# muelea/tuch

Hardware: AMD Instinct MI355X
Metric: SMPLify-DC fit iters/sec at batch 64 (higher is better)
Workload: dtype f32; 1 GPU; configs[1] extended to the full stage-2 step: batch=64/GPU SMPL forward + contact_fitting_loss (L_P/L_C push/pull, winding inside test, segment filter, r2r) + backward + Adam, V=6890 F=13776, float32; bodies_per_gpu=64, global_batch=64, launch=hipGraph replay of the whole step

## Files before the change

tuch_amd/csrc/ray_winding.hip:

```cpp
#include "common.h"
#include "model.h"
#include "workspace.h"
#include "tree_device.h"
#include <stdlib.h>

#pragma clang fp contract(off)

namespace {

constexpr float kPi = 3.14159265358979323846f;
constexpr int kBlock = 256;
constexpr int kRayQueries = 64;
constexpr float kShearX = 0.3217f, kShearY = 0.4331f;
constexpr float kFanX = 0.8191f, kFanY = 0.3467f, kFanZ = 0.4571f;
constexpr int kSlabs = 9;
constexpr int kSlabStride = 10;
constexpr int kNearSlabs = 13;

struct RayElem { float x, y, z, sign; };

__device__ __forceinline__ float shear_x(float x, float z) { return __builtin_fmaf(-kShearX, z, x); }
__device__ __forceinline__ float shear_y(float y, float z) { return __builtin_fmaf(-kShearY, z, y); }

__global__ __launch_bounds__(kBlock) void ray_stream_kernel(
// ... 1 lines not shown
    int V, int L, int Lpad, RayElem* __restrict__ out, uint4* __restrict__ zeroed, size_t zeroed_n)
{
    const int b = blockIdx.y;
    const int p = blockIdx.x * kBlock + threadIdx.x;
    for (size_t g = ((size_t)b * gridDim.x + blockIdx.x) * kBlock + threadIdx.x; g < zeroed_n;
         g += (size_t)gridDim.x * gridDim.y * kBlock)
        zeroed[g] = make_uint4(0u, 0u, 0u, 0u);
    if (p >= Lpad) return;
    RayElem e = {0.f, 0.f, 0.f, 0.f};
    if (p < L) {
        const float* c = verts + ((size_t)b * V + vidx[p]) * 3;
        e.x = shear_x(c[0], c[2]); e.y = shear_y(c[1], c[2]); e.z = c[2]; e.sign = sign[p];
    }
    out[(size_t)b * Lpad + p] = e;
}

__device__ __forceinline__ void slab_project(float x, float y, float z, float (&p)[kSlabs])
{
    p[0] = x; p[1] = y; p[2] = z;
    p[3] = x + y; p[4] = x - y; p[5] = x + z; p[6] = x - z; p[7] = y + z; p[8] = y - z;
}

template <int kCtrl>
__device__ __forceinline__ float dpp_move(float x)
{
    return __int_as_float(__builtin_amdgcn_update_dpp(0, __float_as_int(x), kCtrl, 0xF, 0xF, true));
}
__device__ __forceinline__ float row_min(float v)
{
    v = fminf(v, dpp_move<0xB1>(v));
    v = fminf(v, dpp_move<0x4E>(v));
    v = fminf(v, dpp_move<0x141>(v));
    v = fminf(v, dpp_move<0x140>(v));
    return v;
}

__device__ __forceinline__ uint32_t half_below(float x)
{
    const _Float16 h = (_Float16)x;
    uint32_t u = __builtin_bit_cast(uint16_t, h);
    if ((float)h > x) u = (u & 0x8000u) ? u + 1 : (u == 0 ? 0x8001u : u - 1);
    return u;
}
__device__ __forceinline__ uint32_t half_above(float x)
{
    const _Float16 h = (_Float16)x;
    uint32_t u = __builtin_bit_cast(uint16_t, h);
    if ((float)h < x) u = (u & 0x8000u) ? (u == 0x8000u ? 0x0001u : u - 1) : u + 1;
    return u;
}
__device__ __host__ __forceinline__ size_t near_records_at(int B, int L) { return (size_t)B * kNearSlabs * L; }
__device__ __host__ __forceinline__ size_t near_centres_at(int B, int L) { return near_records_at(B, L) + (size_t)B * L * 8; }

template <bool kPose>
__global__ __launch_bounds__(kBoundsBlock) void ray_leaf_bounds_kernel(
    const RayElem* __restrict__ stream, int T, const TreeNode* __restrict__ nodes, int N,
    const int32_t* __restrict__ height_off, const int32_t* __restrict__ height_nodes, float* __restrict__ bounds,
    const float* __restrict__ verts, const int32_t* __restrict__ vidx, const float* __restrict__ sign, int V, int Lexact,
    RayElem* __restrict__ stream_out, uint4* __restrict__ zeroed, size_t zeroed_n)
{
    const int b = blockIdx.y;
    const RayElem* st = stream + (size_t)b * T;
    const int group = threadIdx.x >> 4, sub = threadIdx.x & 15;
    const int i = height_off[0] + blockIdx.x * (kBoundsBlock / 16) + group;
    const bool real = i < height_off[1];
    const int node = height_nodes[real ? i : height_off[0]];
    const int off = nodes[node].ex_off, len = real ? nodes[node].ex_len : 0;
    if (kPose) {
        for (size_t g = ((size_t)b * gridDim.x + blockIdx.x) * kBoundsBlock + threadIdx.x; g < zeroed_n;
             g += (size_t)gridDim.x * gridDim.y * kBoundsBlock)
            zeroed[g] = make_uint4(0u, 0u, 0u, 0u);
        if (blockIdx.x == 0)
            for (int p = Lexact + (int)threadIdx.x; p < T; p += kBoundsBlock) stream_out[(size_t)b * T + p] = RayElem{0.f, 0.f, 0.f, 0.f};
    }
    float lo[kSlabs], nhi[kSlabs];
#pragma unroll
    for (int k = 0; k < kSlabs; ++k) { lo[k] = 3.0e38f; nhi[k] = 3.0e38f; }
    for (int p = sub; p < len; p += 16) {
        RayElem e;
        if (kPose) {
            const float* c = verts + ((size_t)b * V + vidx[off + p]) * 3;
            e.x = shear_x(c[0], c[2]); e.y = shear_y(c[1], c[2]); e.z = c[2]; e.sign = sign[off + p];
            stream_out[(size_t)b * T + off + p] = e;
        } else {
            e = st[off + p];
        }
        float pr[kSlabs];
        slab_project(e.x, e.y, e.z, pr);
#pragma unroll
        for (int k = 0; k < kSlabs; ++k) { lo[k] = fminf(lo[k], pr[k]); nhi[k] = fminf(nhi[k], -pr[k]); }
    }
#pragma unroll
    for (int k = 0; k < kSlabs; ++k) { lo[k] = row_min(lo[k]); nhi[k] = row_min(nhi[k]); }
    if (real && sub == 0) {
        const int L = height_off[1] - height_off[0], leaf = i - height_off[0];
        float lo_p[kSlabs], hi_p[kSlabs];
#pragma unroll
        for (int k = 0; k < kSlabs; ++k) {
            const float hi = -nhi[k];
            const float pad = 4e-7f * fmaxf(fabsf(lo[k]), fabsf(hi)) + 1e-9f;
            lo_p[k] = lo[k] - pad;
            hi_p[k] = hi + pad;
        }
        float c[3];
        if (kPose) {
            const float* c0 = verts + ((size_t)b * V + vidx[0]) * 3;
            c[0] = shear_x(c0[0], c0[2]); c[1] = shear_y(c0[1], c0[2]); c[2] = c0[2];
        } else {
            const RayElem e0 = st[0];
            c[0] = e0.x; c[1] = e0.y; c[2] = e0.z;
        }
        float pc[kSlabs];
        slab_project(c[0], c[1], c[2], pc);
        uint32_t lo_h[kSlabs], hi_h[kSlabs];
#pragma unroll
        for (int k = 0; k < kSlabs; ++k) {
            const float pad = 4e-6f * (fabsf(lo_p[k]) + fabsf(hi_p[k]) + fabsf(pc[k])) + 1e-7f;
            lo_h[k] = half_below(lo_p[k] - pc[k] - pad);
            hi_h[k] = half_above(hi_p[k] - pc[k] + pad);
        }
        uint4* r = reinterpret_cast<uint4*>(bounds + near_records_at(gridDim.y, L)) + ((size_t)b * L + leaf) * 2;
        r[0] = make_uint4(lo_h[0] | lo_h[1] << 16, lo_h[3] | lo_h[4] << 16, lo_h[6] | lo_h[8] << 16, hi_h[0] | hi_h[1] << 16);
        r[1] = make_uint4(hi_h[2] | hi_h[3] << 16, hi_h[4] | hi_h[5] << 16, hi_h[7] | (uint32_t)leaf << 16, (uint32_t)node);
        if (leaf == 0) *reinterpret_cast<float4*>(bounds + near_centres_at(gridDim.y, L) + (size_t)b * 4) = make_float4(c[0], c[1], c[2], 0.f);
    }
}

struct P3 { float x, y, z; };

__device__ __forceinline__ float edge_fn(const P3& p, const P3& q) { return p.x * q.y - p.y * q.x; }

__device__ __forceinline__ bool left_of(float e, const P3& p, const P3& q)
{
    return e > 0.0f || (e == 0.0f && (p.x < q.x || (p.x == q.x && p.y < q.y)));
}

__device__ __forceinline__ int crossing(const P3& a, const P3& b, const P3& c, float ea, float eb, float ec)
{
    const bool la = left_of(ea, b, c), lb = left_of(eb, c, a), lc = left_of(ec, a, b);
    const bool pos = la && lb && lc, neg = !la && !lb && !lc;
    if (!(pos || neg)) return 0;
    const float numz = ea * a.z + eb * b.z + ec * c.z;
    if (pos) return numz > 0.0f ? 1 : 0;
    return numz < 0.0f ? -1 : 0;
}

__device__ __forceinline__ int crossing_mostly_generic(const P3& a, const P3& b, const P3& c, float ea, float eb, float ec)
{
    const float numz = ea * a.z + eb * b.z + ec * c.z;
    const float mn = __builtin_fminf(__builtin_fminf(ea, eb), ec), mx = __builtin_fmaxf(__builtin_fmaxf(ea, eb), ec);
    int n = (int)(__builtin_fminf(mn, numz) > 0.0f) - (int)(__builtin_fmaxf(mx, numz) < 0.0f);
    const bool tie = (mn * mx == 0.0f) & (numz != 0.0f);
    if (__builtin_amdgcn_ballot_w64(tie)) {
        if (tie) n = crossing(a, b, c, ea, eb, ec);
    }
    return n;
}

template <bool kSkipIncident>
__device__ __forceinline__ int crossing_with_ties(const P3 a, const P3 b, const P3 c, float ea, float eb, float ec)
{
    if (kSkipIncident) {
        const bool za = (a.x == 0.0f) & (a.y == 0.0f) & (a.z == 0.0f);
        const bool zb = (b.x == 0.0f) & (b.y == 0.0f) & (b.z == 0.0f);
        const bool zc = (c.x == 0.0f) & (c.y == 0.0f) & (c.z == 0.0f);
        if (za | zb | zc) return 0;
    }
    return crossing(a, b, c, ea, eb, ec);
}

constexpr uint32_t kSegBias = 0x80808080u;
struct S3 { v2f xy; float z; };
__device__ __forceinline__ float edge_fn(const S3& p, const S3& q)
{
    v2f r;
    asm("v_pk_mul_f32 %0, %1, %2 op_sel:[0,1] op_sel_hi:[1,0]" : "=v"(r) : "v"(p.xy), "v"(q.xy));
    float d;
    asm("v_sub_f32 %0, %1, %2" : "=v"(d) : "v"(r.x), "v"(r.y));
    return d;
}
__device__ __forceinline__ P3 p3(const S3& a) { return P3{a.xy.x, a.xy.y, a.z}; }

template <int A, bool kSkipIncident, bool kSeg>
__device__ __forceinline__ void ray_step(const RayElem el, S3 (&s)[3], float (&e)[3], v2f qxy, float qz, int& count,
                                         int qmask, uint32_t& pa, uint32_t& pb)
{
    constexpr int Bq = (A + 1) % 3, Cq = (A + 2) % 3;
    s[A].xy = (v2f){el.x, el.y} - qxy;
    s[A].z = el.z - qz;
    e[Bq] = edge_fn(s[Cq], s[A]);
    e[Cq] = edge_fn(s[A], s[Bq]);
    const int word = __float_as_int(el.sign);
    if ((word & 0xffffff) != 0) {
        const float numz = __builtin_fmaf(e[A], s[A].z, __builtin_fmaf(e[Cq], s[Cq].z, e[Bq] * s[Bq].z));
        const float mn = __builtin_fminf(__builtin_fminf(e[0], e[1]), e[2]);
        const float mx = __builtin_fmaxf(__builtin_fmaxf(e[0], e[1]), e[2]);
        int c = (int)(__builtin_fminf(mn, numz) > 0.0f) - (int)(__builtin_fmaxf(mx, numz) < 0.0f);
        const bool edge_zero = mn * mx == 0.0f;
        if (__builtin_amdgcn_ballot_w64(edge_zero)) {
            const bool tie = edge_zero & (numz != 0.0f);
            if (__builtin_amdgcn_ballot_w64(tie)) {
                if (tie) c = crossing_with_ties<kSkipIncident>(p3(s[Bq]), p3(s[Cq]), p3(s[A]), e[Bq], e[Cq], e[A]);
            }
        }
        asm("v_mad_i32_i24 %0, %1, %2, %0" : "+v"(count) : "v"(c), "s"(word));
        if (kSeg && ((uint32_t)word >> 24) != 0) {
            const uint32_t t = ((uint32_t)word >> 24) & (uint32_t)qmask;
            if (__builtin_amdgcn_ballot_w64((t != 0) & (c != 0))) {
                uint32_t cs;
                asm("v_mul_i32_i24 %0, %1, %2" : "=v"(cs) : "v"(c), "s"(word));
                pa += cs * (((t & 15u) * 0x00204081u) & 0x01010101u);
                pb += cs * ((((t >> 4) & 15u) * 0x00204081u) & 0x01010101u);
            }
        }
    }
}

template <bool kSkipIncident, bool kSeg>
__device__ __forceinline__ void ray_run(const RayElem* __restrict__ st, int off, int len,
                                        S3 (&s)[3], float (&e)[3], v2f qxy, float qz, int& count,
                                        int qmask, uint32_t& pa, uint32_t& pb)
{
    const RayElem* p = st + off;
    RayElem n0 = p[0], n1 = p[1], n2 = p[2];
    for (int left = len; left > 0; left -= 3, p += 3) {
        asm("" : "+s"(left));
        const RayElem e0 = n0, e1 = n1, e2 = n2;
        n0 = p[3]; n1 = p[4]; n2 = p[5];
        ray_step<0, kSkipIncident, kSeg>(e0, s, e, qxy, qz, count, qmask, pa, pb);
        ray_step<1, kSkipIncident, kSeg>(e1, s, e, qxy, qz, count, qmask, pa, pb);
        ray_step<2, kSkipIncident, kSeg>(e2, s, e, qxy, qz, count, qmask, pa, pb);
    }
}

constexpr int kFallbackChunks = 8;

__device__ __forceinline__ float wave_min(float v) { return wave_min_uniform(v); }
__device__ __forceinline__ float wave_max(float v) { return wave_max_uniform(v); }


__device__ __forceinline__ float lo_minus(uint32_t s, float q)
{
    float d;
    asm("v_fma_mix_f32 %0, %1, 1.0, -%2 op_sel_hi:[1,0,0]" : "=v"(d) : "v"(s), "v"(q));
    return d;
}
__device__ __forceinline__ float hi_minus(uint32_t s, float q)
{
    float d;
    asm("v_fma_mix_f32 %0, %1, 1.0, -%2 op_sel:[1,0,0] op_sel_hi:[1,0,0]" : "=v"(d) : "v"(s), "v"(q));
    return d;
}
__device__ __forceinline__ float minus_lo(float q, uint32_t s)
{
    float d;
    asm("v_fma_mix_f32 %0, -%1, 1.0, %2 op_sel_hi:[1,0,0]" : "=v"(d) : "v"(s), "v"(q));
    return d;
}
__device__ __forceinline__ float minus_hi(float q, uint32_t s)
{
    float d;
    asm("v_fma_mix_f32 %0, -%1, 1.0, %2 op_sel:[1,0,0] op_sel_hi:[1,0,0]" : "=v"(d) : "v"(s), "v"(q));
    return d;
}
__device__ __forceinline__ float max3(float a, float b, float c)
{
    float d;
    asm("v_max3_f32 %0, %1, %2, %3" : "=v"(d) : "v"(a), "v"(b), "v"(c));
    return d;
}

template <bool kVerts, int kWaves>
__global__ __launch_bounds__(64 * kWaves) void ray_near_kernel(
    const float* __restrict__ pts, const TreeNode* __restrict__ nodes, const float* __restrict__ bounds, int N,
    int num_leaves, const int32_t* __restrict__ qperm,
    const int32_t* __restrict__ counts, int Q, int qblocks, RayEntry* __restrict__ lists, int32_t* __restrict__ list_len,
    int32_t* __restrict__ leaf_cnt,
    unsigned long long* __restrict__ stats)
{
    __builtin_amdgcn_s_setprio(3);
    const int qb = blockIdx.x, b = blockIdx.y, lane = threadIdx.x & 63;
    const int wave = kWaves > 1 ? __builtin_amdgcn_readfirstlane(threadIdx.x >> 6) : 0;
    __shared__ uint4 queue[64 * kWaves][2];
    __shared__ float range[16];
// ... 237 lines not shown
    const bool overflow = total_pairs > cap || total_tiles > max_tiles;
    if (lane == 0 && blockIdx.y == 0) body[b] = RayBody{overflow ? fallback_tiles : total_tiles, overflow ? 1 : 0};
    if (overflow) return;
    {
        int off = sp - npairs, tile = st - ntile;
        for (int l = l0; l < l1; ++l) {
            const int c = cnt[l];
            off_s[l] = off;
            tile_s[l] = tile;
            off += c;
            tile += (c + 63) >> 6;
        }
        int ent = sq - nent;
        for (int q = q0; q < q1; ++q) { blk[q] = ent; ent += len[q]; }
        if (lane == 0) blk[qblocks] = total;
    }
    __syncthreads();
    for (int l = (int)blockIdx.y + (int)gridDim.y * lane; l < num_leaves; l += (int)gridDim.y * 64) {
        const TreeNode nd = nodes[leaf_nodes[l]];
        const int ex_off = nd.ex_off, ex_len = nd.ex_len;
        const int c = cnt[l], off = off_s[l];
        RayTile* out = tiles + (size_t)b * max_tiles + tile_s[l];
        for (int k = 0; k < c; k += 64) *out++ = RayTile{ex_off, ex_len, off + k, min(64, c - k)};
    }
    int32_t* fill = leaf_fill + (size_t)b * num_leaves;
    int32_t* out = pairs + (size_t)b * cap;
    for (int base = (int)blockIdx.y * 64; base < total; base += (int)gridDim.y * 64) {
        const int g = base + lane;
        RayEntry e = RayEntry{0, 0, 0u, 0u};
        int dst = 0, qb = 0;
        if (g < total) {
            int lo = 0, hi = qblocks;
            while (hi - lo > 1) {
                const int mid = (lo + hi) >> 1;
                if (blk[mid] <= g) lo = mid; else hi = mid;
            }
            qb = lo;
            e = lists[((size_t)b * qblocks + qb) * list_stride + (g - blk[qb])];
            dst = off_s[e.leaf] + atomicAdd(&fill[e.leaf], __builtin_popcount(e.mask_lo) + __builtin_popcount(e.mask_hi));
        }
        const int m = min(64, total - base);
        for (int k = 0; k < m; ++k) {
            const uint32_t lo = __builtin_amdgcn_readlane(e.mask_lo, k), hi = __builtin_amdgcn_readlane(e.mask_hi, k);
            const int d = __builtin_amdgcn_readlane(dst, k), q = __builtin_amdgcn_readlane(qb, k);
            const unsigned long long mask = ((unsigned long long)hi << 32) | lo;
            if ((mask >> lane) & 1ull)
                out[d + __builtin_popcountll(mask & ((1ull << lane) - 1ull))] = q * kRayQueries + lane;
        }
    }
}

template <bool kVerts, bool kCount, bool kSeg>
__global__ __launch_bounds__(64) void ray_leaf_kernel(
    const float* __restrict__ pts, const RayElem* __restrict__ stream, const RayTile* __restrict__ tiles,
    const RayBody* __restrict__ body, const int32_t* __restrict__ pairs, const RayEntry* __restrict__ lists,
    const int32_t* __restrict__ list_len, const TreeNode* __restrict__ nodes, int num_leaves,
    const int32_t* __restrict__ qperm, const int32_t* __restrict__ counts, int Q, int T, int qblocks, int num_bodies,
    int cap, int max_tiles, int32_t* __restrict__ count, unsigned long long* __restrict__ stats,
    const int32_t* __restrict__ vmask, int32_t* __restrict__ seg_count)
{
    const int lane = threadIdx.x;
    struct Work { int b, off, len, slot, qmask; bool active; float qx, qy, qz; };
    int b_cur = blockIdx.x, base = 0, g = blockIdx.y;
    auto fetch = [&]() {
        Work w;
        w.b = -1; w.off = w.len = w.slot = 0; w.qmask = 0; w.active = false; w.qx = w.qy = w.qz = 0.0f;
        while (b_cur < num_bodies) {
            const int b = b_cur;
            const int nt = __builtin_amdgcn_readfirstlane(body[b].tiles);
            if (g >= base + nt) { base += nt; b_cur += gridDim.x; continue; }
            const int t = g - base;
            g += gridDim.y;
            const float* pb = pts + (size_t)b * Q * 3;
            w.b = b;
            int i0;
            if (!__builtin_amdgcn_readfirstlane(body[b].overflow)) {
                const RayTile tile = tiles[(size_t)b * max_tiles + t];
                const int n = __builtin_amdgcn_readfirstlane(tile.n), first = __builtin_amdgcn_readfirstlane(tile.first);
                w.active = lane < n;
                w.slot = pairs[(size_t)b * cap + first + (w.active ? lane : 0)];
                i0 = kVerts ? qperm[w.slot] : w.slot;
                w.off = __builtin_amdgcn_readfirstlane(tile.ex_off);
                w.len = __builtin_amdgcn_readfirstlane(tile.ex_len);
            } else {
                const int nq = kVerts ? Q : (counts ? counts[b] : Q);
                w.slot = (t / kFallbackChunks) * kRayQueries + lane;
                w.active = w.slot < nq;
                i0 = kVerts ? qperm[w.slot] : min(w.slot, nq - 1);
                w.off = t;
                w.len = -1;
            }
            w.qz = pb[3 * i0 + 2];
            w.qx = shear_x(pb[3 * i0], w.qz);
            w.qy = shear_y(pb[3 * i0 + 1], w.qz);
            if (kSeg) w.qmask = vmask[w.slot];
            break;
        }
        return w;
    };
    int walked = 0;
    Work next = fetch();
    while (next.b >= 0) {
        const Work w = next;
        next = fetch();
        S3 s[3];
        float e[3];
#pragma unroll
        for (int k = 0; k < 3; ++k) { s[k].xy = (v2f){0.0f, 0.0f}; s[k].z = 0.0f; e[k] = 0.0f; }
        const v2f qxy = {w.qx, w.qy};
        int crossings = 0;
        uint32_t pa = kSegBias, pb = kSegBias;
        const RayElem* st = stream + (size_t)w.b * T;
        if (w.len >= 0) {
            ray_run<kVerts, kSeg>(st, w.off, w.len, s, e, qxy, w.qz, crossings, w.qmask, pa, pb);
            if (kCount) walked += w.len;
        } else {
            const int qb = w.off / kFallbackChunks, c = w.off % kFallbackChunks;
            const int cnt = __builtin_amdgcn_readfirstlane(list_len[(size_t)w.b * qblocks + qb]);
            const RayEntry* list = lists + ((size_t)w.b * qblocks + qb) * num_leaves;
            for (int j = c; j < cnt; j += kFallbackChunks) {
                const TreeNode nd = nodes[__builtin_amdgcn_readfirstlane(list[j].node)];
                ray_run<kVerts, kSeg>(st, nd.ex_off, nd.ex_len, s, e, qxy, w.qz, crossings, w.qmask, pa, pb);
                if (kCount) walked += nd.ex_len;
            }
        }
        if (w.active && crossings != 0) atomicAdd(&count[((size_t)w.b * qblocks) * kRayQueries + w.slot], crossings);
        if (kSeg && w.active && (pa != kSegBias || pb != kSegBias)) {
            int32_t* sc = seg_count + 2 * (((size_t)w.b * qblocks) * kRayQueries + w.slot);
            if (pa != kSegBias) atomicAdd(sc, (int32_t)(pa - kSegBias));
            if (pb != kSegBias) atomicAdd(sc + 1, (int32_t)(pb - kSegBias));
        }
    }
    if (kCount && lane == 0) atomicAdd(stats, (unsigned long long)walked);
}

__device__ __forceinline__ float fast_atan2(float y, float x)
{
    const float ax = __builtin_fabsf(x), ay = __builtin_fabsf(y);
    const float mx = __builtin_fmaxf(__builtin_fmaxf(ax, ay), 1e-37f);
    const float t = __builtin_fminf(ax, ay) / mx;
    const float s = t * t;
    float p = 0.0024567253421992064f;
    p = p * s + -0.014401361346244812f;
    p = p * s + 0.03978123143315315f;
    p = p * s + -0.07234857976436615f;
    p = p * s + 0.10498946160078049f;
    p = p * s + -0.14161229133605957f;
    p = p * s + 0.19985906779766083f;
    p = p * s + -0.33332598209381104f;
    p = p * s + 0.9999998807907104f;
    float v = p * t;
    v = ay > ax ? 1.57079632679489661923f - v : v;
    v = x < 0.0f ? kPi - v : v;
    return __builtin_copysignf(v, y);
}

__device__ __forceinline__ float half_solid_angle(const P3& a, const P3& b, const P3& c)
{
    const float na = __builtin_sqrtf(a.x * a.x + a.y * a.y + a.z * a.z);
    const float nb = __builtin_sqrtf(b.x * b.x + b.y * b.y + b.z * b.z);
    const float nc = __builtin_sqrtf(c.x * c.x + c.y * c.y + c.z * c.z);
    const float cx = b.y * c.z - b.z * c.y, cy = b.z * c.x - b.x * c.z, cz = b.x * c.y - b.y * c.x;
    const float num = a.x * cx + a.y * cy + a.z * cz;
    const float dab = a.x * b.x + a.y * b.y + a.z * b.z;
    const float dbc = b.x * c.x + b.y * c.y + b.z * c.z;
    const float dac = a.x * c.x + a.y * c.y + a.z * c.z;
    const float den = na * nb * nc + dab * nc + dac * nb + dbc * na;
    return fast_atan2(num, den);
}

__device__ __forceinline__ void cone_term(const P3& us, const P3& sb, const P3& sc, const P3& u, const P3& pb, const P3& pc,
                                          int& crossings, float& half)
{
    const float ea = edge_fn(sb, sc), eb = edge_fn(sc, us), ec = edge_fn(us, sb);
    const float d = ea * us.z + eb * sb.z + ec * sc.z;
    const bool la = left_of(ea, sb, sc), lb = left_of(eb, sc, us), lc = left_of(ec, us, sb);
    const bool front = d >= 0.0f;
    crossings = (la & lb & lc) ? (int)front : ((!la & !lb & !lc) ? -(int)!front : 0);
    const float nu = __builtin_sqrtf(u.x * u.x + u.y * u.y + u.z * u.z);
    const float nb = __builtin_sqrtf(pb.x * pb.x + pb.y * pb.y + pb.z * pb.z);
    const float nc = __builtin_sqrtf(pc.x * pc.x + pc.y * pc.y + pc.z * pc.z);
    const float cx = pb.y * pc.z - pb.z * pc.y, cy = pb.z * pc.x - pb.x * pc.z, cz = pb.x * pc.y - pb.y * pc.x;
    const float num = __builtin_fabsf(u.x * cx + u.y * cy + u.z * cz);
// ... 319 lines not shown
        h += h1;
        c += c1;
    };
    const int e0 = active ? link_off[qq] : 0, e1 = active ? link_off[qq + 1] : 0;
    constexpr int kLongLinks = 16;
    if (e1 - e0 <= kLongLinks) {
        for (int e = e0; e < e1; e += 2) {
            int id[4];
            float pp[4][3];
#pragma unroll
            for (int u = 0; u < 4; ++u) id[u] = link[2 * min(e + (u >> 1), e1 - 1) + (u & 1)];
#pragma unroll
            for (int u = 0; u < 4; ++u) {
                const float* p = id[u] < V ? vb + 3 * (size_t)id[u] : cb + 3 * (size_t)(id[u] - V);
                pp[u][0] = p[0]; pp[u][1] = p[1]; pp[u][2] = p[2];
            }
#pragma unroll
            for (int h = 0; h < 2; ++h)
                if (e + h < e1) cone(pp[2 * h], pp[2 * h + 1], vx, vy, vz, qx, qy, half_sum, n);
        }
    }
    unsigned long long todo = __builtin_amdgcn_ballot_w64(e1 - e0 > kLongLinks);
    const int lane = threadIdx.x & 63;
    while (todo) {
        const int src = __builtin_ctzll(todo);
        todo &= todo - 1;
        const int le0 = __builtin_amdgcn_readlane(e0, src), le1 = __builtin_amdgcn_readlane(e1, src);
        const float lvx = __shfl(vx, src), lvy = __shfl(vy, src), lvz = __shfl(vz, src);
        const float lqx = __shfl(qx, src), lqy = __shfl(qy, src);
        float h = 0.0f;
        int cr = 0;
        for (int e = le0 + lane; e < le1; e += 64) {
            const int i0 = link[2 * e], i1 = link[2 * e + 1];
            const float* p0 = i0 < V ? vb + 3 * (size_t)i0 : cb + 3 * (size_t)(i0 - V);
            const float* p1 = i1 < V ? vb + 3 * (size_t)i1 : cb + 3 * (size_t)(i1 - V);
            const float a0[3] = {p0[0], p0[1], p0[2]}, a1[3] = {p1[0], p1[1], p1[2]};
            cone(a0, a1, lvx, lvy, lvz, lqx, lqy, h, cr);
        }
#pragma unroll
        for (int m = 32; m >= 1; m >>= 1) { h += __shfl_xor(h, m); cr += __shfl_xor(cr, m); }
        if (lane == src) { half_sum += h; n += cr; }
    }
    if (!active) return;
    const float w = (float)n - half_sum * (0.5f / kPi);
    const size_t o = (size_t)b * Qs_total + qq;
    if (seg_w) seg_w[o] = w;
    if (seg_ext) seg_ext[o] = w <= thresh;
    if (exterior && !(w <= thresh)) exterior[(size_t)b * V + v] = 1;
}

inline size_t align256(size_t x) { return (x + 255) & ~(size_t)255; }

struct RayLayout {
    size_t stream, bounds, lists, list_len, zeroed, zeroed_bytes, leaf_cnt, leaf_fill, count, leaf_off, tiles, body, pairs,
        stats, total;
    int T, qblocks, cap, max_tiles, workers, columns;
    size_t seg_count;
};

constexpr int kSegFusedMaxQ = 4096;
constexpr int kSegFusedMaxCaps = 8;

template <int kWaves>
__device__ __forceinline__ void seg_fused_caps(const float* __restrict__ vb, const int32_t* __restrict__ cap_off,
                                               const int32_t* __restrict__ cap_vidx, int c_lo, int c_hi, float* s_caps)
{
    const int lane = threadIdx.x & 63, wave = threadIdx.x >> 6;
    for (int c = c_lo + wave; c < c_hi; c += kWaves) {
        float sx = 0.f, sy = 0.f, sz = 0.f;
        const int beg = cap_off[c], end = cap_off[c + 1];
        for (int k = beg + lane; k < end; k += 64) {
            const float* p = vb + 3 * cap_vidx[k];
            sx += p[0]; sy += p[1]; sz += p[2];
        }
#pragma unroll
        for (int o = 32; o > 0; o >>= 1) { sx += __shfl_down(sx, o, 64); sy += __shfl_down(sy, o, 64); sz += __shfl_down(sz, o, 64); }
        if (lane == 0) {
            const float inv = 1.0f / (float)(end - beg);
            s_caps[3 * (c - c_lo)] = sx * inv; s_caps[3 * (c - c_lo) + 1] = sy * inv; s_caps[3 * (c - c_lo) + 2] = sz * inv;
        }
    }
}

constexpr int kSegOneBlock = 512, kSegOneWaves = kSegOneBlock / 64, kSegOneChunk = 256, kSegOneZ = 8;
constexpr int kSegOneOwn = kSegFusedMaxQ / kSegOneZ;
#ifdef TUCH_SEG_CLOCKS
__device__ unsigned long long g_seg_clocks[8192][8];
#define SEG_CLOCK(i) do { if (threadIdx.x == 0) { const int blk = (blockIdx.z * gridDim.y + blockIdx.y) * gridDim.x + blockIdx.x; if (blk < 8192) g_seg_clocks[blk][i] = __builtin_amdgcn_s_memrealtime(); } } while (0)
extern "C" int tuch_debug_seg_clocks(unsigned long long* out)
{
    return hipMemcpyFromSymbol(out, HIP_SYMBOL(g_seg_clocks), sizeof(unsigned long long) * 8192 * 8) == hipSuccess ? TUCH_OK : TUCH_ERR_HIP;
}
#else
#define SEG_CLOCK(i) do { } while (0)
#endif

__global__ __launch_bounds__(kSegOneBlock) void segment_one_kernel(
    const float* __restrict__ verts, const uint8_t* __restrict__ body_flags, uint8_t* __restrict__ exterior,
    const int32_t* __restrict__ seg_q_off, const int32_t* __restrict__ seg_q_vidx,
    const int32_t* __restrict__ cap_range, const int32_t* __restrict__ cap_off, const int32_t* __restrict__ cap_vidx,
    const int32_t* __restrict__ ent_off, const int32_t* __restrict__ ent,
    const int32_t* __restrict__ link_off, const int32_t* __restrict__ link, const int32_t* __restrict__ leaf_counts,
    const int32_t* __restrict__ vpos, int slots, int V, float thresh)
{
    __shared__ int32_t s_list[kSegFusedMaxQ];
    __shared__ int32_t s_cnt[kSegOneOwn];
    __shared__ float s_half[kSegOneOwn];
// ... 190 lines not shown
}

int tuch_ray_segment_flags_one(const tuch_contact_model* m, const float* verts, const uint8_t* body_flags,
                               const int32_t* leaf_counts, int B, float thresh, uint8_t* exterior, hipStream_t s)
{
    hipLaunchKernelGGL(segment_one_kernel, dim3(m->num_segments, B, kSegOneZ), dim3(kSegOneBlock), 0, s, verts, body_flags, exterior,
                       (const int32_t*)m->seg_q_off, (const int32_t*)m->seg_q_vidx, (const int32_t*)m->seg_cap_range,
                       (const int32_t*)m->cap_off, (const int32_t*)m->cap_vidx, (const int32_t*)m->seg_cap_off,
                       (const int32_t*)m->seg_cap_ent, (const int32_t*)m->seg_link_off, (const int32_t*)m->seg_link, leaf_counts,
                       (const int32_t*)m->seg_vpos, 2 * m->tree_qblocks * kRayQueries, m->V, thresh);
    return tuch_check_launch("tuch_ray_segment_flags_one");
}

bool tuch_ray_available(const tuch_contact_model* m)
{
    if (!m || m->tree_nodes <= 0 || !m->ring_off || m->tree_exact_len <= 0) return false;
    if (m->tree_leaves > 65535) return false;
    return m->opt.winding_ray != 0;
}

static int ray_pair_cap(const tuch_contact_model* m) { return m->opt.ray_pair_cap < 1 ? 1 : m->opt.ray_pair_cap; }

static RayLayout full_layout(const tuch_contact_model* m, int B, int Q, bool verts)
{
    RayLayout l;
    l.qblocks = verts ? 2 * m->tree_qblocks : ceil_div(Q, kRayQueries);
    l.T = ceil_div(m->tree_exact_len, 3) * 3 + 6;
    const int L = m->tree_leaves;
    const long cap = (long)ray_pair_cap(m) * Q;
    l.cap = (int)(cap < 0x3fffffffL ? cap : 0x3fffffffL);
    l.max_tiles = l.cap / 64 + L;
    if (l.max_tiles < l.qblocks * kFallbackChunks) l.max_tiles = l.qblocks * kFallbackChunks;
    l.columns = B < 8 ? B : 8;
    const int waves = m->opt.ray_waves > 0 ? m->opt.ray_waves : 32768;
    l.workers = waves / l.columns > 0 ? waves / l.columns : 1;
    size_t o = 0;
    l.stream = tuch_ws_take(o, (size_t)B * l.T * sizeof(RayElem));
    l.bounds = tuch_ws_take(o, (size_t)B * m->tree_nodes * 2 * kSlabStride * sizeof(float));
    l.lists = tuch_ws_take(o, (size_t)B * l.qblocks * L * sizeof(RayEntry));
    l.list_len = tuch_ws_take(o, (size_t)B * l.qblocks * sizeof(int32_t));
    l.zeroed = o;
    l.leaf_cnt = tuch_ws_take(o, (size_t)B * L * sizeof(int32_t), false);
    l.leaf_fill = tuch_ws_take(o, (size_t)B * L * sizeof(int32_t), false);
    l.count = tuch_ws_take(o, (size_t)B * l.qblocks * kRayQueries * sizeof(int32_t), false);
    l.seg_count = o;
    if (verts && m->seg_elem_mask) o += align256(2 * (size_t)B * l.qblocks * kRayQueries * sizeof(int32_t));
    l.zeroed_bytes = o - l.zeroed;
    (void)tuch_ws_take(o, 0);
    l.leaf_off = tuch_ws_take(o, (size_t)B * L * sizeof(int32_t));
    l.tiles = tuch_ws_take(o, (size_t)B * l.max_tiles * sizeof(RayTile));
    l.body = tuch_ws_take(o, (size_t)B * sizeof(RayBody));
    l.pairs = tuch_ws_take(o, (size_t)B * l.cap * sizeof(int32_t));
    l.stats = tuch_ws_take(o, 256);
    l.total = o;
    return l;
}

void tuch_ray_layout_touch(const tuch_contact_model* m, int B, int Q)
{
    (void)full_layout(m, B, Q > 0 ? Q : m->V, Q <= 0);
}

size_t tuch_ray_workspace_bytes(const tuch_contact_model* m, int B, int Q)
{
    if (!m || m->tree_nodes <= 0 || B <= 0) return 0;
    const size_t a = full_layout(m, B, m->V, true).total;
    const size_t b = Q > 0 ? full_layout(m, B, Q, false).total : 0;
    return a > b ? a : b;
}

static void launch_ray_boxes(const tuch_contact_model* m, const RayLayout& l, const float* verts, int B, char* ws, hipStream_t s,
                             bool one_launch)
{
    RayElem* st = (RayElem*)(ws + l.stream);
    float* bounds = (float*)(ws + l.bounds);
    if (one_launch && m->tree_leaf_runs_tile) {
        hipLaunchKernelGGL(ray_leaf_bounds_kernel<true>, dim3(ceil_div(m->tree_leaves, kBoundsBlock / 16), B), dim3(kBoundsBlock), 0,
                           s, (const RayElem*)st, l.T, (const TreeNode*)m->tree_node, m->tree_nodes,
                           (const int32_t*)m->tree_height_off, (const int32_t*)m->tree_height_nodes, bounds, verts,
                           (const int32_t*)m->tree_vidx, (const float*)m->tree_sign_word, m->V, m->tree_exact_len, st,
                           (uint4*)(ws + l.zeroed), l.zeroed_bytes / sizeof(uint4));
        return;
    }
    hipLaunchKernelGGL(ray_stream_kernel, dim3(ceil_div(l.T, kBlock), B), dim3(kBlock), 0, s, verts,
                       (const int32_t*)m->tree_vidx, (const float*)m->tree_sign_word, m->V, m->tree_exact_len, l.T, st,
                       (uint4*)(ws + l.zeroed), l.zeroed_bytes / sizeof(uint4));
    hipLaunchKernelGGL(ray_leaf_bounds_kernel<false>, dim3(ceil_div(m->tree_leaves, kBoundsBlock / 16), B), dim3(kBoundsBlock), 0, s,
                       (const RayElem*)st, l.T, (const TreeNode*)m->tree_node, m->tree_nodes,
                       (const int32_t*)m->tree_height_off, (const int32_t*)m->tree_height_nodes, bounds,
                       (const float*)nullptr, (const int32_t*)nullptr, (const float*)nullptr, 0, 0, (RayElem*)nullptr,
                       (uint4*)nullptr, (size_t)0);
}

template <bool kVerts>
static int launch_ray_counts(const tuch_contact_model* m, const RayLayout& l, const float* verts, const float* queries,
                             const int32_t* counts, int B, int Q, char* ws, hipStream_t s, unsigned long long* stats)
{
    launch_ray_boxes(m, l, verts, B, ws, s, kVerts);
    const int L = m->tree_leaves;
    const TreeNode* nodes = (const TreeNode*)m->tree_node;
    const int32_t* leaf_nodes = (const int32_t*)m->tree_height_nodes;
    const int32_t* qperm = kVerts ? (const int32_t*)m->tree_qperm : nullptr;
    RayEntry* lists = (RayEntry*)(ws + l.lists);
    int32_t* list_len = (int32_t*)(ws + l.list_len);
    int32_t* leaf_cnt = (int32_t*)(ws + l.leaf_cnt);
    int32_t* leaf_off = (int32_t*)(ws + l.leaf_off);
    RayTile* tiles = (RayTile*)(ws + l.tiles);
    RayBody* body = (RayBody*)(ws + l.body);
    int32_t* pairs = (int32_t*)(ws + l.pairs);
    if ((long)l.qblocks * B <= 2048)
        hipLaunchKernelGGL((ray_near_kernel<kVerts, 4>), dim3(l.qblocks, B), dim3(256), 0, s, queries, nodes,
                           (const float*)(ws + l.bounds), m->tree_nodes, L, qperm, counts, Q, l.qblocks, lists, list_len,
                           leaf_cnt, stats);
    else
        hipLaunchKernelGGL((ray_near_kernel<kVerts, 1>), dim3(l.qblocks, B), dim3(64), 0, s, queries, nodes,
                           (const float*)(ws + l.bounds), m->tree_nodes, L, qperm, counts, Q, l.qblocks, lists, list_len,
                           leaf_cnt, stats);
    const size_t tf_lds = (2 * (size_t)L + l.qblocks + 1) * sizeof(int32_t);
    if (l.qblocks <= kFillMaxBlocks && tf_lds <= 48u * 1024)
        hipLaunchKernelGGL(ray_tiles_fill_kernel, dim3(B, std::min(256, std::max(kFillSplit, 2048 / B))), dim3(kTilesFillBlock), tf_lds, s, (const int32_t*)leaf_cnt,
                           nodes, leaf_nodes, L, l.cap, l.max_tiles, l.qblocks * kFallbackChunks, tiles, body,
                           (const RayEntry*)lists, (const int32_t*)list_len, l.qblocks, (int32_t*)(ws + l.leaf_fill), pairs, L);
    else {
    hipLaunchKernelGGL(ray_tiles_kernel, dim3(B), dim3(kTilesBlock), 0, s, (const int32_t*)leaf_cnt, nodes, leaf_nodes, L, l.cap,
                       l.max_tiles, l.qblocks * kFallbackChunks, leaf_off, tiles, body);
    hipLaunchKernelGGL(ray_fill_kernel, dim3(l.qblocks, B), dim3(64), 0, s, (const RayEntry*)lists, (const int32_t*)list_len,
                       (const RayBody*)body, (const int32_t*)leaf_off, L, l.qblocks, l.cap, (int32_t*)(ws + l.leaf_fill), pairs);
    }
    const dim3 grid(l.columns, l.workers);
    const bool seg = kVerts && m->seg_elem_mask;
    const int32_t* vmask = (const int32_t*)m->seg_vmask;
    int32_t* seg_count = (int32_t*)(ws + l.seg_count);
#define TUCH_LAUNCH_RAY_LEAF(COUNT, SEG)                                                                                      \
    hipLaunchKernelGGL((ray_leaf_kernel<kVerts, COUNT, SEG>), grid, dim3(64), 0, s, queries, (const RayElem*)(ws + l.stream),  \
                       (const RayTile*)tiles, (const RayBody*)body, (const int32_t*)pairs, (const RayEntry*)lists,            \
                       (const int32_t*)list_len, nodes, L, qperm, counts, Q, l.T, l.qblocks, B, l.cap, l.max_tiles,           \
                       (int32_t*)(ws + l.count), stats, vmask, seg_count)
    if (stats) {
        if (seg) TUCH_LAUNCH_RAY_LEAF(true, kVerts); else TUCH_LAUNCH_RAY_LEAF(true, false);
    } else {
        if (seg) TUCH_LAUNCH_RAY_LEAF(false, kVerts); else TUCH_LAUNCH_RAY_LEAF(false, false);
    }
#undef TUCH_LAUNCH_RAY_LEAF
    return TUCH_OK;
}

int tuch_ray_exterior_verts(const tuch_contact_model* m, const float* verts, int B, float thresh, uint8_t* exterior,
                            float* w, void* workspace, hipStream_t s, unsigned long long* stats_host, uint8_t* exterior_copy)
{
    const RayLayout l = full_layout(m, B, m->V, true);
    char* ws = (char*)workspace;
    unsigned long long* stats = stats_host ? (unsigned long long*)(ws + l.stats) : nullptr;
    if (stats && hipMemsetAsync(stats, 0, 4 * sizeof(unsigned long long), s) != hipSuccess) return TUCH_ERR_HIP;
    const int rc = launch_ray_counts<true>(m, l, verts, verts, nullptr, B, m->V, ws, s, stats);
    if (rc != TUCH_OK) return rc;
    if (w || exterior)
        hipLaunchKernelGGL(ray_finalize_verts_kernel, dim3(ceil_div(m->V, kBlock), B), dim3(kBlock), 0, s, verts,
                           (const int32_t*)(ws + l.count), (const int32_t*)m->tree_qperm, (const int32_t*)m->ring_off,
                           (const int32_t*)m->ring_vidx, m->V, l.qblocks * kRayQueries, thresh, w, exterior, exterior_copy);
    if (stats_host) {
        RayBody bodies[8];
        const int nb = B < 8 ? B : 8;
        if (hipMemcpyAsync(stats_host, stats, 3 * sizeof(unsigned long long), hipMemcpyDeviceToHost, s) != hipSuccess ||
            hipMemcpyAsync(bodies, ws + l.body, nb * sizeof(RayBody), hipMemcpyDeviceToHost, s) != hipSuccess ||
            hipStreamSynchronize(s) != hipSuccess)
            return TUCH_ERR_HIP;
        unsigned long long tiles = 0;
        for (int b = 0; b < nb; ++b) tiles += bodies[b].tiles;
        stats_host[3] = tiles * B / nb;
    }
    return tuch_check_launch("tuch_ray_exterior_verts");
}

const int32_t* tuch_ray_segment_counts(const tuch_contact_model* m, int B, const void* workspace)
{
    if (!m->seg_elem_mask) return nullptr;
    return (const int32_t*)((const char*)workspace + full_layout(m, B, m->V, true).seg_count);
}

int tuch_ray_exterior_points(const tuch_contact_model* m, const float* verts, const float* points, const int32_t* counts,
                             int B, int Q, float thresh, uint8_t* exterior, float* w, void* workspace, hipStream_t s)
{
    const RayLayout l = full_layout(m, B, Q, false);
    char* ws = (char*)workspace;
    const int rc = launch_ray_counts<false>(m, l, verts, points, counts, B, Q, ws, s, nullptr);
    if (rc != TUCH_OK) return rc;
    hipLaunchKernelGGL(ray_finalize_points_kernel, dim3(ceil_div(Q, kBlock), B), dim3(kBlock), 0, s,
                       (const int32_t*)(ws + l.count), counts, Q, l.qblocks * kRayQueries, thresh, w, exterior);
// ... 41 lines not shown
```

Before: 152,800 body-fit iterations/s.

## Filter ray-winding triangles by 2D boxes and queue survivors for exact tests

```diff
diff --git a/tuch_amd/csrc/ray_winding.hip b/tuch_amd/csrc/ray_winding.hip
--- a/tuch_amd/csrc/ray_winding.hip
+++ b/tuch_amd/csrc/ray_winding.hip
@@ -77,12 +77,30 @@
 __device__ __host__ __forceinline__ size_t near_records_at(int B, int L) { return (size_t)B * kNearSlabs * L; }
 __device__ __host__ __forceinline__ size_t near_centres_at(int B, int L) { return near_records_at(B, L) + (size_t)B * L * 8; }
 
+constexpr float kBoxRange = 16.0f;
+constexpr float kBoxPad = 0x1p-13f;
+constexpr float kBoxSliver = 0x1p-14f;
+__device__ __forceinline__ float4 ray_elem_box(const RayElem& p0, const RayElem& p1, const RayElem& p2)
+{
+    const float inf = __builtin_inff();
+    if ((__float_as_int(p2.sign) & 0xffffff) == 0) return make_float4(inf, -inf, inf, -inf);
+    const float x0 = fminf(fminf(p0.x, p1.x), p2.x), x1 = fmaxf(fmaxf(p0.x, p1.x), p2.x);
+    const float y0 = fminf(fminf(p0.y, p1.y), p2.y), y1 = fmaxf(fmaxf(p0.y, p1.y), p2.y);
+    const float ax = p1.x - p0.x, ay = p1.y - p0.y, bx = p2.x - p0.x, by = p2.y - p0.y;
+    const float area2 = fabsf(ax * by - ay * bx);
+    const float edge = fmaxf(fmaxf(x1 - x0, y1 - y0), 0.0f);
+    const bool in_range = fmaxf(fmaxf(fabsf(x0), fabsf(x1)), fmaxf(fabsf(y0), fabsf(y1))) <= kBoxRange;
+    const bool solid = area2 > kBoxSliver * 1.4142137f * edge;
+    if (!in_range || !solid) return make_float4(-inf, inf, -inf, inf);
+    return make_float4(x0 - kBoxPad, x1 + kBoxPad, y0 - kBoxPad, y1 + kBoxPad);
+}
+
 template <bool kPose>
 __global__ __launch_bounds__(kBoundsBlock) void ray_leaf_bounds_kernel(
     const RayElem* __restrict__ stream, int T, const TreeNode* __restrict__ nodes, int N,
     const int32_t* __restrict__ height_off, const int32_t* __restrict__ height_nodes, float* __restrict__ bounds,
     const float* __restrict__ verts, const int32_t* __restrict__ vidx, const float* __restrict__ sign, int V, int Lexact,
-    RayElem* __restrict__ stream_out, uint4* __restrict__ zeroed, size_t zeroed_n)
+    RayElem* __restrict__ stream_out, uint4* __restrict__ zeroed, size_t zeroed_n, float4* __restrict__ boxes)
 {
     const int b = blockIdx.y;
     const RayElem* st = stream + (size_t)b * T;
@@ -98,18 +116,26 @@
         if (blockIdx.x == 0)
             for (int p = Lexact + (int)threadIdx.x; p < T; p += kBoundsBlock) stream_out[(size_t)b * T + p] = RayElem{0.f, 0.f, 0.f, 0.f};
     }
+    if (blockIdx.x == 0)
+        for (int p = Lexact + (int)threadIdx.x; p < T; p += kBoundsBlock)
+            boxes[(size_t)b * T + p] = make_float4(__builtin_inff(), -__builtin_inff(), __builtin_inff(), -__builtin_inff());
+    auto posed = [&](int p) {
+        RayElem e;
+        if (kPose) {
+            const float* c = verts + ((size_t)b * V + vidx[p]) * 3;
+            e.x = shear_x(c[0], c[2]); e.y = shear_y(c[1], c[2]); e.z = c[2]; e.sign = sign[p];
+        } else {
+            e = st[p];
+        }
+        return e;
+    };
     float lo[kSlabs], nhi[kSlabs];
 #pragma unroll
     for (int k = 0; k < kSlabs; ++k) { lo[k] = 3.0e38f; nhi[k] = 3.0e38f; }
     for (int p = sub; p < len; p += 16) {
-        RayElem e;
-        if (kPose) {
-            const float* c = verts + ((size_t)b * V + vidx[off + p]) * 3;
-            e.x = shear_x(c[0], c[2]); e.y = shear_y(c[1], c[2]); e.z = c[2]; e.sign = sign[off + p];
-            stream_out[(size_t)b * T + off + p] = e;
-        } else {
-            e = st[off + p];
-        }
+        const RayElem e = posed(off + p);
+        if (kPose) stream_out[(size_t)b * T + off + p] = e;
+        boxes[(size_t)b * T + off + p] = ray_elem_box(posed(off + max(p - 2, 0)), posed(off + max(p - 1, 0)), e);
         float pr[kSlabs];
         slab_project(e.x, e.y, e.z, pr);
 #pragma unroll
@@ -194,7 +220,6 @@
     return crossing(a, b, c, ea, eb, ec);
 }
 
-constexpr uint32_t kSegBias = 0x80808080u;
 struct S3 { v2f xy; float z; };
 __device__ __forceinline__ float edge_fn(const S3& p, const S3& q)
 {
@@ -206,55 +231,157 @@
 }
 __device__ __forceinline__ P3 p3(const S3& a) { return P3{a.xy.x, a.xy.y, a.z}; }
 
-template <int A, bool kSkipIncident, bool kSeg>
-__device__ __forceinline__ void ray_step(const RayElem el, S3 (&s)[3], float (&e)[3], v2f qxy, float qz, int& count,
-                                         int qmask, uint32_t& pa, uint32_t& pb)
-{
-    constexpr int Bq = (A + 1) % 3, Cq = (A + 2) % 3;
-    s[A].xy = (v2f){el.x, el.y} - qxy;
-    s[A].z = el.z - qz;
-    e[Bq] = edge_fn(s[Cq], s[A]);
-    e[Cq] = edge_fn(s[A], s[Bq]);
-    const int word = __float_as_int(el.sign);
-    if ((word & 0xffffff) != 0) {
-        const float numz = __builtin_fmaf(e[A], s[A].z, __builtin_fmaf(e[Cq], s[Cq].z, e[Bq] * s[Bq].z));
-        const float mn = __builtin_fminf(__builtin_fminf(e[0], e[1]), e[2]);
-        const float mx = __builtin_fmaxf(__builtin_fmaxf(e[0], e[1]), e[2]);
-        int c = (int)(__builtin_fminf(mn, numz) > 0.0f) - (int)(__builtin_fmaxf(mx, numz) < 0.0f);
-        const bool edge_zero = mn * mx == 0.0f;
-        if (__builtin_amdgcn_ballot_w64(edge_zero)) {
-            const bool tie = edge_zero & (numz != 0.0f);
-            if (__builtin_amdgcn_ballot_w64(tie)) {
-                if (tie) c = crossing_with_ties<kSkipIncident>(p3(s[Bq]), p3(s[Cq]), p3(s[A]), e[Bq], e[Cq], e[A]);
-            }
-        }
-        asm("v_mad_i32_i24 %0, %1, %2, %0" : "+v"(count) : "v"(c), "s"(word));
-        if (kSeg && ((uint32_t)word >> 24) != 0) {
-            const uint32_t t = ((uint32_t)word >> 24) & (uint32_t)qmask;
-            if (__builtin_amdgcn_ballot_w64((t != 0) & (c != 0))) {
-                uint32_t cs;
-                asm("v_mul_i32_i24 %0, %1, %2" : "=v"(cs) : "v"(c), "s"(word));
-                pa += cs * (((t & 15u) * 0x00204081u) & 0x01010101u);
-                pb += cs * ((((t >> 4) & 15u) * 0x00204081u) & 0x01010101u);
-            }
-        }
-    }
-}
+constexpr int kRingSize = 128;
+struct RayQueue {
+    uint32_t ring[kRingSize];
+    int32_t cross[kRayQueries];
+    uint32_t seg[2][kRayQueries];
+    float4 box[64];
+    RayElem elem[64];
+};
+constexpr int kBoxChunk = 60;
+struct RayLane { float fx, fy, qx, qy, qz; int qmask; bool active; };
 
 template <bool kSkipIncident, bool kSeg>
-__device__ __forceinline__ void ray_run(const RayElem* __restrict__ st, int off, int len,
-                                        S3 (&s)[3], float (&e)[3], v2f qxy, float qz, int& count,
-                                        int qmask, uint32_t& pa, uint32_t& pb)
-{
-    const RayElem* p = st + off;
-    RayElem n0 = p[0], n1 = p[1], n2 = p[2];
-    for (int left = len; left > 0; left -= 3, p += 3) {
-        asm("" : "+s"(left));
-        const RayElem e0 = n0, e1 = n1, e2 = n2;
-        n0 = p[3]; n1 = p[4]; n2 = p[5];
-        ray_step<0, kSkipIncident, kSeg>(e0, s, e, qxy, qz, count, qmask, pa, pb);
-        ray_step<1, kSkipIncident, kSeg>(e1, s, e, qxy, qz, count, qmask, pa, pb);
-        ray_step<2, kSkipIncident, kSeg>(e2, s, e, qxy, qz, count, qmask, pa, pb);
+__device__ __forceinline__ void ray_exact(RayQueue& q, uint32_t& head, int n, const RayLane& me, int lane)
+{
+    __syncthreads();
+    const bool valid = lane < n;
+    const uint32_t ent = q.ring[(head + (uint32_t)lane) & (kRingSize - 1)];
+    head += (uint32_t)n;
+    const int r = (int)(ent & 63u);
+    const uint32_t k = min(ent >> 6, (uint32_t)(kBoxChunk + 1));
+    const float ox = __int_as_float(__builtin_amdgcn_ds_bpermute(r << 2, __float_as_int(me.qx)));
+    const float oy = __int_as_float(__builtin_amdgcn_ds_bpermute(r << 2, __float_as_int(me.qy)));
+    const float oz = __int_as_float(__builtin_amdgcn_ds_bpermute(r << 2, __float_as_int(me.qz)));
+    const int om = kSeg ? __builtin_amdgcn_ds_bpermute(r << 2, me.qmask) : 0;
+    const RayElem el0 = q.elem[k], el1 = q.elem[k + 1], el2 = q.elem[k + 2];
+    const v2f oxy = {ox, oy};
+    S3 s0, s1, s2;
+    s0.xy = (v2f){el0.x, el0.y} - oxy; s0.z = el0.z - oz;
+    s1.xy = (v2f){el1.x, el1.y} - oxy; s1.z = el1.z - oz;
+    s2.xy = (v2f){el2.x, el2.y} - oxy; s2.z = el2.z - oz;
+    const float e0 = edge_fn(s1, s2), e1 = edge_fn(s2, s0), e2 = edge_fn(s0, s1);
+    const float numz = __builtin_fmaf(e2, s2.z, __builtin_fmaf(e1, s1.z, e0 * s0.z));
+    const float mn = __builtin_fminf(__builtin_fminf(e0, e1), e2);
+    const float mx = __builtin_fmaxf(__builtin_fmaxf(e0, e1), e2);
+    int c = (int)(__builtin_fminf(mn, numz) > 0.0f) - (int)(__builtin_fmaxf(mx, numz) < 0.0f);
+    const bool tie = (mn * mx == 0.0f) & (numz != 0.0f);
+    if (__builtin_amdgcn_ballot_w64(tie)) {
+        if (tie) c = crossing_with_ties<kSkipIncident>(p3(s0), p3(s1), p3(s2), e0, e1, e2);
+    }
+    const int word = __float_as_int(el2.sign);
+    const int cs = c * ((word << 8) >> 8);
+    if (valid && cs != 0) {
+        atomicAdd(&q.cross[r], cs);
+        if (kSeg) {
+            const uint32_t t = ((uint32_t)word >> 24) & (uint32_t)om;
+            if (t & 15u) atomicAdd(&q.seg[0][r], (uint32_t)cs * (((t & 15u) * 0x00204081u) & 0x01010101u));
+            if (t >> 4) atomicAdd(&q.seg[1][r], (uint32_t)cs * ((((t >> 4) & 15u) * 0x00204081u) & 0x01010101u));
+        }
+    }
+}
+
+__device__ __forceinline__ uint32_t lanes_below(unsigned long long m)
+{
+    return __builtin_amdgcn_mbcnt_hi((uint32_t)(m >> 32), __builtin_amdgcn_mbcnt_lo((uint32_t)m, 0u));
+}
+
+template <int K>
+__device__ __forceinline__ void ray_filter(const float4 box, unsigned long long all, float fx, float fy, uint32_t& mask)
+{
+    asm volatile("v_cmpx_ngt_f32 vcc, %[lox], %[fx]\n\t"
+                 "v_cmpx_nlt_f32 vcc, %[hix], %[fx]\n\t"
+                 "v_cmpx_ngt_f32 vcc, %[loy], %[fy]\n\t"
+                 "v_cmpx_nlt_f32 vcc, %[hiy], %[fy]\n\t"
+                 "v_or_b32 %[m], %[bit], %[m]\n\t"
+                 "s_mov_b64 exec, %[sv]"
+                 : [m] "+v"(mask)
+                 : [lox] "v"(box.x), [hix] "v"(box.y), [loy] "v"(box.z), [hiy] "v"(box.w), [bit] "n"(1u << K), [sv] "s"(all),
+                   [fx] "v"(fx), [fy] "v"(fy)
+                 : "vcc");
+}
+
+template <bool kSkipIncident, bool kSeg>
+__device__ __forceinline__ void ray_append(uint32_t mask, int base, RayQueue& q, uint32_t& head, uint32_t& tail,
+                                           const RayLane& me, int lane)
+{
+    unsigned long long m;
+    while ((m = __builtin_amdgcn_ballot_w64(mask != 0u)) != 0ull) {
+        if (mask != 0u) {
+            const int k = __builtin_ctz(mask);
+            mask &= mask - 1u;
+            q.ring[(tail + lanes_below(m)) & (kRingSize - 1)] = ((uint32_t)(base + k) << 6) | (uint32_t)lane;
+        }
+        tail += (uint32_t)__builtin_popcountll(m);
+        if (tail - head >= 64u) ray_exact<kSkipIncident, kSeg>(q, head, 64, me, lane);
+    }
+}
+
+template <bool kSkipIncident, bool kSeg>
+__device__ __forceinline__ void ray_run(const RayElem* __restrict__ st, const float4* __restrict__ boxes, int off, int len, int T,
+                                        RayQueue& q, uint32_t& head, uint32_t& tail, const RayLane& me, int lane,
+                                        bool have_pre, const float4 pre, const RayElem pre_el)
+{
+    const unsigned long long all = __builtin_amdgcn_read_exec();
+    for (int c0 = 0; c0 < len; c0 += kBoxChunk) {
+    float4 mine = pre;
+    RayElem mine_el = pre_el;
+    if (!(have_pre && c0 == 0)) {
+        mine = boxes[min(off + c0 + lane, T - 1)];
+        mine_el = st[min(max(off + c0 - 2 + lane, 0), T - 1)];
+    }
+    while (tail != head) ray_exact<kSkipIncident, kSeg>(q, head, (int)min(tail - head, 64u), me, lane);
+    __syncthreads();
+    q.box[lane] = mine;
+    q.elem[lane] = mine_el;
+    __syncthreads();
+    const float4* p = q.box;
+    float4 n0 = p[0], n1 = p[1], n2 = p[2];
+    int at = 0, left = min(len - c0, kBoxChunk);
+#define TUCH_RAY_TRIPLE(J)                                                         \
+    {                                                                              \
+        const float4 b0 = n0, b1 = n1, b2 = n2;                                    \
+        n0 = p[3]; n1 = p[4]; n2 = p[5];                                           \
+        ray_filter<3 * J>(b0, all, me.fx, me.fy, mask);                            \
+        ray_filter<3 * J + 1>(b1, all, me.fx, me.fy, mask);                        \
+        ray_filter<3 * J + 2>(b2, all, me.fx, me.fy, mask);                        \
+        left -= 3; p += 3;                                                         \
+        asm("" : "+s"(left));                                                      \
+    }
+    while (left > 0) {
+        uint32_t mask = 0u;
+        do {
+            TUCH_RAY_TRIPLE(0) if (left <= 0) break;
+            TUCH_RAY_TRIPLE(1) if (left <= 0) break;
+            TUCH_RAY_TRIPLE(2) if (left <= 0) break;
+            TUCH_RAY_TRIPLE(3) if (left <= 0) break;
+            TUCH_RAY_TRIPLE(4) if (left <= 0) break;
+            TUCH_RAY_TRIPLE(5) if (left <= 0) break;
+            TUCH_RAY_TRIPLE(6) if (left <= 0) break;
+            TUCH_RAY_TRIPLE(7) if (left <= 0) break;
+            TUCH_RAY_TRIPLE(8) if (left <= 0) break;
+            TUCH_RAY_TRIPLE(9)
+        } while (false);
+        if (!me.active) mask = 0u;
+        ray_append<kSkipIncident, kSeg>(mask, at, q, head, tail, me, lane);
+        at += 30;
+    }
+    }
+#undef TUCH_RAY_TRIPLE
+}
+
+template <bool kSkipIncident, bool kSeg>
+__device__ __forceinline__ void ray_flush(RayQueue& q, uint32_t& head, uint32_t tail, const RayLane& me, int lane,
+                                          int& crossings, uint32_t& pa, uint32_t& pb)
+{
+    while (tail != head) ray_exact<kSkipIncident, kSeg>(q, head, (int)min(tail - head, 64u), me, lane);
+    __syncthreads();
+    crossings = q.cross[lane];
+    q.cross[lane] = 0;
+    if (kSeg) {
+        pa = q.seg[0][lane]; pb = q.seg[1][lane];
+        q.seg[0][lane] = 0u; q.seg[1][lane] = 0u;
     }
 }
 
@@ -598,19 +725,21 @@
 
 template <bool kVerts, bool kCount, bool kSeg>
 __global__ __launch_bounds__(64) void ray_leaf_kernel(
-    const float* __restrict__ pts, const RayElem* __restrict__ stream, const RayTile* __restrict__ tiles,
-    const RayBody* __restrict__ body, const int32_t* __restrict__ pairs, const RayEntry* __restrict__ lists,
+    const float* __restrict__ pts, const RayElem* __restrict__ stream, const float4* __restrict__ boxes,
+    const RayTile* __restrict__ tiles, const RayBody* __restrict__ body, const int32_t* __restrict__ pairs, const RayEntry* __restrict__ lists,
     const int32_t* __restrict__ list_len, const TreeNode* __restrict__ nodes, int num_leaves,
     const int32_t* __restrict__ qperm, const int32_t* __restrict__ counts, int Q, int T, int qblocks, int num_bodies,
     int cap, int max_tiles, int32_t* __restrict__ count, unsigned long long* __restrict__ stats,
     const int32_t* __restrict__ vmask, int32_t* __restrict__ seg_count)
 {
     const int lane = threadIdx.x;
-    struct Work { int b, off, len, slot, qmask; bool active; float qx, qy, qz; };
+    struct Work { int b, off, len, slot, qmask; bool active; float qx, qy, qz; float4 pre; RayElem pre_el; };
     int b_cur = blockIdx.x, base = 0, g = blockIdx.y;
     auto fetch = [&]() {
         Work w;
         w.b = -1; w.off = w.len = w.slot = 0; w.qmask = 0; w.active = false; w.qx = w.qy = w.qz = 0.0f;
+        w.pre = make_float4(0.0f, 0.0f, 0.0f, 0.0f);
+        w.pre_el = RayElem{0.0f, 0.0f, 0.0f, 0.0f};
         while (b_cur < num_bodies) {
             const int b = b_cur;
             const int nt = __builtin_amdgcn_readfirstlane(body[b].tiles);
@@ -628,6 +757,8 @@
                 i0 = kVerts ? qperm[w.slot] : w.slot;
                 w.off = __builtin_amdgcn_readfirstlane(tile.ex_off);
                 w.len = __builtin_amdgcn_readfirstlane(tile.ex_len);
+                w.pre = boxes[(size_t)b * T + min(w.off + lane, T - 1)];
+                w.pre_el = stream[(size_t)b * T + min(max(w.off - 2 + lane, 0), T - 1)];
             } else {
                 const int nq = kVerts ? Q : (counts ? counts[b] : Q);
                 w.slot = (t / kFallbackChunks) * kRayQueries + lane;
@@ -645,20 +776,26 @@
         return w;
     };
     int walked = 0;
+    __shared__ RayQueue queue;
+    queue.cross[lane] = 0;
+    queue.seg[0][lane] = 0u; queue.seg[1][lane] = 0u;
+    queue.ring[lane] = 0u; queue.ring[lane + 64] = 0u;
+    uint32_t head = 0u, tail = 0u;
     Work next = fetch();
     while (next.b >= 0) {
         const Work w = next;
         next = fetch();
-        S3 s[3];
-        float e[3];
-#pragma unroll
-        for (int k = 0; k < 3; ++k) { s[k].xy = (v2f){0.0f, 0.0f}; s[k].z = 0.0f; e[k] = 0.0f; }
-        const v2f qxy = {w.qx, w.qy};
+        RayLane me;
+        me.qx = w.qx; me.qy = w.qy; me.qz = w.qz; me.qmask = w.qmask; me.active = w.active;
+        const bool near = (__builtin_fabsf(w.qx) <= kBoxRange) & (__builtin_fabsf(w.qy) <= kBoxRange);
+        me.fx = near ? w.qx : __builtin_nanf("");
+        me.fy = near ? w.qy : __builtin_nanf("");
         int crossings = 0;
-        uint32_t pa = kSegBias, pb = kSegBias;
+        uint32_t pa = 0u, pb = 0u;
         const RayElem* st = stream + (size_t)w.b * T;
+        const float4* bx = boxes + (size_t)w.b * T;
         if (w.len >= 0) {
-            ray_run<kVerts, kSeg>(st, w.off, w.len, s, e, qxy, w.qz, crossings, w.qmask, pa, pb);
+            ray_run<kVerts, kSeg>(st, bx, w.off, w.len, T, queue, head, tail, me, lane, true, w.pre, w.pre_el);
             if (kCount) walked += w.len;
         } else {
             const int qb = w.off / kFallbackChunks, c = w.off % kFallbackChunks;
@@ -666,15 +803,16 @@
             const RayEntry* list = lists + ((size_t)w.b * qblocks + qb) * num_leaves;
             for (int j = c; j < cnt; j += kFallbackChunks) {
                 const TreeNode nd = nodes[__builtin_amdgcn_readfirstlane(list[j].node)];
-                ray_run<kVerts, kSeg>(st, nd.ex_off, nd.ex_len, s, e, qxy, w.qz, crossings, w.qmask, pa, pb);
+                ray_run<kVerts, kSeg>(st, bx, nd.ex_off, nd.ex_len, T, queue, head, tail, me, lane, false, w.pre, w.pre_el);
                 if (kCount) walked += nd.ex_len;
             }
         }
+        ray_flush<kVerts, kSeg>(queue, head, tail, me, lane, crossings, pa, pb);
         if (w.active && crossings != 0) atomicAdd(&count[((size_t)w.b * qblocks) * kRayQueries + w.slot], crossings);
-        if (kSeg && w.active && (pa != kSegBias || pb != kSegBias)) {
+        if (kSeg && w.active && (pa != 0u || pb != 0u)) {
             int32_t* sc = seg_count + 2 * (((size_t)w.b * qblocks) * kRayQueries + w.slot);
-            if (pa != kSegBias) atomicAdd(sc, (int32_t)(pa - kSegBias));
-            if (pb != kSegBias) atomicAdd(sc + 1, (int32_t)(pb - kSegBias));
+            if (pa != 0u) atomicAdd(sc, (int32_t)pa);
+            if (pb != 0u) atomicAdd(sc + 1, (int32_t)pb);
         }
     }
     if (kCount && lane == 0) atomicAdd(stats, (unsigned long long)walked);
@@ -1100,7 +1238,7 @@
 inline size_t align256(size_t x) { return (x + 255) & ~(size_t)255; }
 
 struct RayLayout {
-    size_t stream, bounds, lists, list_len, zeroed, zeroed_bytes, leaf_cnt, leaf_fill, count, leaf_off, tiles, body, pairs,
+    size_t stream, boxes, bounds, lists, list_len, zeroed, zeroed_bytes, leaf_cnt, leaf_fill, count, leaf_off, tiles, body, pairs,
         stats, total;
     int T, qblocks, cap, max_tiles, workers, columns;
     size_t seg_count;
@@ -1397,6 +1535,7 @@
     l.body = tuch_ws_take(o, (size_t)B * sizeof(RayBody));
     l.pairs = tuch_ws_take(o, (size_t)B * l.cap * sizeof(int32_t));
     l.stats = tuch_ws_take(o, 256);
+    l.boxes = tuch_ws_take(o, (size_t)B * l.T * sizeof(float4));
     l.total = o;
     return l;
 }
@@ -1424,7 +1563,7 @@
                            s, (const RayElem*)st, l.T, (const TreeNode*)m->tree_node, m->tree_nodes,
                            (const int32_t*)m->tree_height_off, (const int32_t*)m->tree_height_nodes, bounds, verts,
                            (const int32_t*)m->tree_vidx, (const float*)m->tree_sign_word, m->V, m->tree_exact_len, st,
-                           (uint4*)(ws + l.zeroed), l.zeroed_bytes / sizeof(uint4));
+                           (uint4*)(ws + l.zeroed), l.zeroed_bytes / sizeof(uint4), (float4*)(ws + l.boxes));
         return;
     }
     hipLaunchKernelGGL(ray_stream_kernel, dim3(ceil_div(l.T, kBlock), B), dim3(kBlock), 0, s, verts,
@@ -1433,8 +1572,8 @@
     hipLaunchKernelGGL(ray_leaf_bounds_kernel<false>, dim3(ceil_div(m->tree_leaves, kBoundsBlock / 16), B), dim3(kBoundsBlock), 0, s,
                        (const RayElem*)st, l.T, (const TreeNode*)m->tree_node, m->tree_nodes,
                        (const int32_t*)m->tree_height_off, (const int32_t*)m->tree_height_nodes, bounds,
-                       (const float*)nullptr, (const int32_t*)nullptr, (const float*)nullptr, 0, 0, (RayElem*)nullptr,
-                       (uint4*)nullptr, (size_t)0);
+                       (const float*)nullptr, (const int32_t*)nullptr, (const float*)nullptr, 0, m->tree_exact_len, (RayElem*)nullptr,
+                       (uint4*)nullptr, (size_t)0, (float4*)(ws + l.boxes));
 }
 
 template <bool kVerts>
@@ -1478,7 +1617,7 @@
     int32_t* seg_count = (int32_t*)(ws + l.seg_count);
 #define TUCH_LAUNCH_RAY_LEAF(COUNT, SEG)                                                                                      \
     hipLaunchKernelGGL((ray_leaf_kernel<kVerts, COUNT, SEG>), grid, dim3(64), 0, s, queries, (const RayElem*)(ws + l.stream),  \
-                       (const RayTile*)tiles, (const RayBody*)body, (const int32_t*)pairs, (const RayEntry*)lists,            \
+                       (const float4*)(ws + l.boxes), (const RayTile*)tiles, (const RayBody*)body, (const int32_t*)pairs, (const RayEntry*)lists,            \
                        (const int32_t*)list_len, nodes, L, qperm, counts, Q, l.T, l.qblocks, B, l.cap, l.max_tiles,           \
                        (int32_t*)(ws + l.count), stats, vmask, seg_count)
     if (stats) {
```

Measured after the change: 159,200 body-fit iterations/s, median of 6. 4.2% higher.
